# bdaiinstitute/judo

Measured on AMD Instinct MI355X. Metric: rollouts/sec + plan-step ms, leap_cube MPPI 65536xH64, higher is better.
Workload: dtype f32

## Files before the change

include/judo_amd.h:

```cpp
#ifndef JUDO_AMD_H
#define JUDO_AMD_H

#include <stddef.h>
#include <stdint.h>

#ifdef __cplusplus
extern "C" {
#endif

typedef struct jh_model jh_model;

enum jh_status {
  JH_OK = 0,
  JH_ERR_INVALID = -1,
  JH_ERR_HIP = -2,
  JH_ERR_UNSUPPORTED = -3,
  JH_ERR_BLOB = -4
};

enum jh_task_kind { JH_TASK_CARTPOLE = 0, JH_TASK_CYLINDER_PUSH = 1, JH_TASK_LEAP_CUBE = 2, JH_TASK_FR3_PICK = 3 };
enum jh_spline_kind { JH_SPLINE_ZERO = 0, JH_SPLINE_LINEAR = 1, JH_SPLINE_CUBIC = 3 };

#define JH_MAX_TASK_PARAMS 32
#define JH_MAX_KNOT_DIM 512
// ... 14 lines not shown
int jh_model_set_contact_capacity(jh_model* m, int contacts);

int jh_model_build(const jh_model* m, int* out );

int jh_model_fr3_build(const jh_model* m, int* out );

int jh_model_trace_layout(const jh_model* m, int* out );
int jh_trace_gather(const float* rec_in , int k, int stride_in, int n_offset, int n_local, const float* trace , int row_floats,
                    int colmajor, float* rec_out , void* stream);

int jh_model_limits(const jh_model* m, int* out );
int jh_model_max_fused_knots(const jh_model* m, int H);
int jh_model_one_launch_max_knots(const jh_model* m, int H);
int jh_model_set_plan_step_launches(jh_model* m, int launches);
int jh_model_set_rollout_schedule(jh_model* m, int mode);

int jh_upload_async(void* dst_device, const void* src_host, size_t nbytes, void* stream);
int jh_download_wait(void* dst_host, const void* src_device, size_t nbytes, void* stream);
int jh_download_begin(void* dst_host, const void* src_device, size_t nbytes, void* stream);
int jh_download_end(void);

int jh_rollout_cost(const jh_model* m, const float* x0, const float* nominal, const float* noise, int ldn, const float* sigma,
                    const float* W, const float* ctrl_lo_hi, const float* task_params, int phase, int N, int n_offset, int H, int K,
                    float* costs, float* knots_out, void* stream);
int jh_rollout_cost_traced(const jh_model* m, const float* x0, const float* nominal, const float* noise, int ldn, const float* sigma,
                    const float* W, const float* ctrl_lo_hi, const float* task_params, int phase, int N, int n_offset, int H, int K,
                    float* costs, float* knots_out, float* trace , void* stream);

int jh_rollout_materialize(const jh_model* m, const float* x0, int x0_batched, const float* controls, int N, int H, float* states,
                           float* sensors, void* stream);
// ... 99 lines not shown
```

judo_amd/_lib.py:

```python

from __future__ import annotations

import ctypes as C
import os

_HERE = os.path.dirname(os.path.abspath(__file__))
LIB_PATH = os.environ.get("JUDO_AMD_LIB") or os.path.join(_HERE, "libjudo_amd.so")

_lib: C.CDLL | None = None

f32p = C.c_void_p

_SIGNATURES = {
    "jh_last_error": (C.c_char_p, []),
    "jh_version": (C.c_int, []),
    "jh_model_create": (C.c_int, [C.c_void_p, C.c_size_t, C.c_int, C.POINTER(C.c_void_p)]),
    "jh_model_destroy": (None, [C.c_void_p]),
    "jh_model_dims": (C.c_int, [C.c_void_p, C.POINTER(C.c_int)]),
    "jh_model_stats": (C.c_int, [C.c_void_p, C.POINTER(C.c_int), C.c_int]),
    "jh_model_set_kernel": (C.c_int, [C.c_void_p, C.c_int]),
    "jh_model_limits": (C.c_int, [C.c_void_p, C.POINTER(C.c_int)]),
    "jh_register_xcheck": (C.c_int, [C.c_void_p]),
    "jh_model_max_fused_knots": (C.c_int, [C.c_void_p, C.c_int]),
    "jh_model_one_launch_max_knots": (C.c_int, [C.c_void_p, C.c_int]),
    "jh_model_set_plan_step_launches": (C.c_int, [C.c_void_p, C.c_int]),
    "jh_model_set_rollout_schedule": (C.c_int, [C.c_void_p, C.c_int]),
    "jh_model_set_self_collision": (C.c_int, [C.c_void_p, C.c_int]),
    "jh_model_set_contact_capacity": (C.c_int, [C.c_void_p, C.c_int]),
    "jh_model_build": (C.c_int, [C.c_void_p, C.POINTER(C.c_int)]),
    "jh_model_fr3_build": (C.c_int, [C.c_void_p, C.POINTER(C.c_int)]),
    "jh_model_trace_layout": (C.c_int, [C.c_void_p, C.POINTER(C.c_int)]),
    "jh_trace_gather": (C.c_int, [C.c_void_p, C.c_int, C.c_int, C.c_int, C.c_int, C.c_void_p, C.c_int, C.c_int, C.c_void_p, C.c_void_p]),
    "jh_upload_async": (C.c_int, [C.c_void_p, C.c_void_p, C.c_size_t, C.c_void_p]),
    "jh_download_wait": (C.c_int, [C.c_void_p, C.c_void_p, C.c_size_t, C.c_void_p]),
    "jh_download_begin": (C.c_int, [C.c_void_p, C.c_void_p, C.c_size_t, C.c_void_p]),
    "jh_download_end": (C.c_int, []),
    "jh_rollout_cost": (C.c_int, [C.c_void_p, f32p, f32p, f32p, C.c_int, f32p, f32p, f32p, f32p, C.c_int, C.c_int, C.c_int, C.c_int, C.c_int, f32p, f32p, C.c_void_p]),
    "jh_rollout_cost_traced": (C.c_int, [C.c_void_p, f32p, f32p, f32p, C.c_int, f32p, f32p, f32p, f32p, C.c_int, C.c_int, C.c_int, C.c_int, C.c_int, f32p, f32p, f32p, C.c_void_p]),
    "jh_rollout_materialize": (C.c_int, [C.c_void_p, f32p, C.c_int, f32p, C.c_int, C.c_int, f32p, f32p, C.c_void_p]),
    "jh_task_reward": (C.c_int, [C.c_void_p, f32p, f32p, f32p, f32p, C.c_int, C.c_int, C.c_int, f32p, C.c_void_p]),
    "jh_noise_normal": (C.c_int, [C.c_ulonglong, C.c_uint, C.c_int, C.c_int, C.c_int, f32p, C.c_int, C.c_void_p]),
# ... 98 lines not shown
```

judo_amd/csrc/jh_api.hip:

```cpp
#include <algorithm>
#include <cmath>
#include <cstdlib>
#include <cstring>

#include "jh_internal.h"
#include "jh_update_dev.h"

static thread_local char g_err[512] = "";

void jh_set_error(const char* fmt, ...) {
  va_list ap;
  va_start(ap, fmt);
  vsnprintf(g_err, sizeof(g_err), fmt, ap);
  va_end(ap);
}

extern "C" const char* jh_last_error(void) { return g_err; }
extern "C" int jh_version(void) { return 100; }

static int image_cylinders(const jh_blob_header& h, const float* F, const int* I) {
  constexpr int HEADER = 24, BODY_I = 6, BODY_F = 32, BLOCK_I = 4, DOF_F = 20, ACT_I = 2, ACT_F = 8, GEOM_I = 2, GEOM_F = 20, GF_RBOUND = 15;
  if (h.nint < (uint32_t)HEADER || h.nfloat < (uint32_t)HEADER) return 0;
  const long NM = I[0], NBLK = I[1], nv = I[2], nu = I[4], NG = I[5];
  if (NM < 0 || NBLK < 0 || nv < 0 || nu < 0 || NG < 0) return 0;
// ... 106 lines not shown
    std::vector<int> I((const int*)(q + 4 * (size_t)h.nfloat), (const int*)(q + 4 * (size_t)h.nfloat) + h.nint);
    cylinders = image_cylinders(h, F.data(), I.data());
    if (cylinders < 0) return JH_ERR_BLOB;
    if (h.kind == JH_TASK_LEAP_CUBE && image_pair_tables(h, I.data()) < 0) return JH_ERR_BLOB;
    if (cylinders > 0 && h.kind != JH_TASK_LEAP_CUBE) { jh_set_error("model_create: %d cylinder geoms, and only the leap kernel has a cylinder build", cylinders); return JH_ERR_BLOB; }
    if (h.kind == JH_TASK_FR3_PICK) {
      arm_pairs = image_arm_pairs(h, I.data());
      if (arm_pairs < 0) return JH_ERR_BLOB;
    }
  }
  JH_HIP(hipSetDevice(device));
  jh_model* m = new jh_model();
  m->device = device; m->kind = (int)h.kind; m->nq = h.nq; m->nv = h.nv; m->nu = h.nu; m->ns = h.ns; m->ntaskparam = h.ntaskparam;
  m->nf = h.nfloat; m->ni = h.nint; m->d_f = nullptr; m->d_i = nullptr; m->d_stats = nullptr; m->kernel_gen = (h.kind == JH_TASK_LEAP_CUBE || h.kind == JH_TASK_FR3_PICK) ? 3 : 2; m->self_collision = 1; m->contact_capacity = cylinders > 0 ? 64 : 48; m->cylinders = cylinders; m->arm_pairs = arm_pairs;
  { const char* e = getenv("JUDO_AMD_ROLLOUT_SCHEDULE"); m->rollout_schedule = (e && (e[0] == '1' || e[0] == '2')) ? e[0] - '0' : 0; }
  { const char* e = getenv("JUDO_AMD_PLAN_STEP_LAUNCHES"); m->plan_step_launches = (e && e[0] == '2') ? 2 : 0; }
  const char* p = (const char*)blob + sizeof(h);
  m->h_f.assign((const float*)p, (const float*)p + h.nfloat);
  m->h_i.assign((const int*)(p + 4 * (size_t)h.nfloat), (const int*)(p + 4 * (size_t)h.nfloat) + h.nint);
  {
    hipMemPool_t pool = nullptr; int dev = 0;
    if (hipGetDevice(&dev) == hipSuccess && hipDeviceGetDefaultMemPool(&pool, dev) == hipSuccess && pool) {
      unsigned long long keep = ~0ull;
      (void)hipMemPoolSetAttribute(pool, hipMemPoolAttrReleaseThreshold, &keep);
    }
  }
  hipError_t e = hipMalloc(&m->d_f, 4 * (m->nf ? m->nf : 1));
  if (e == hipSuccess) e = hipMalloc(&m->d_i, 4 * (m->ni ? m->ni : 1));
  if (e == hipSuccess) e = hipMalloc(&m->d_stats, JH_NSTATS * sizeof(int));
  if (e == hipSuccess) e = hipMemset(m->d_stats, 0, JH_NSTATS * sizeof(int));
// ... 161 lines not shown
  const int k = JH_MAX_KNOT_DIM / (m->nu > 0 ? m->nu : 1), lds_k = jh_simple_one_launch_max_knots(m, H);
  return k < lds_k ? k : lds_k;
}

extern "C" int jh_model_set_plan_step_launches(jh_model* m, int launches) {
  JH_REQUIRE(m != nullptr && launches >= 0 && launches <= 2, "model_set_plan_step_launches: launches must be 0 (automatic), 1 or 2");
  JH_REQUIRE(launches != 1 || m->kind == JH_TASK_CARTPOLE || m->kind == JH_TASK_CYLINDER_PUSH, "model_set_plan_step_launches: only the closed-form models have a one-launch plan step");
  m->plan_step_launches = launches;
  return JH_OK;
}

extern "C" int jh_model_set_rollout_schedule(jh_model* m, int mode) {
  JH_REQUIRE(m != nullptr && mode >= 0 && mode <= 2, "model_set_rollout_schedule: mode must be 0 (automatic), 1 (static grid) or 2 (persistent waves wherever the kernel has them)");
  m->rollout_schedule = mode;
  return JH_OK;
}

extern "C" int jh_upload_async(void* dst, const void* src, size_t nbytes, void* stream) {
  JH_REQUIRE(dst && src, "upload_async: null pointer");
  JH_HIP(hipMemcpyAsync(dst, src, nbytes, hipMemcpyHostToDevice, (hipStream_t)stream));
  return JH_OK;
}

extern "C" int jh_download_wait(void* dst, const void* src, size_t nbytes, void* stream) {
  JH_REQUIRE(dst && src, "download_wait: null pointer");
  JH_HIP(hipMemcpyAsync(dst, src, nbytes, hipMemcpyDeviceToHost, (hipStream_t)stream));
  JH_HIP(hipStreamSynchronize((hipStream_t)stream));
  return JH_OK;
}

// ... 231 lines not shown
static int model_set_member(const char* who, const jh_model* m0, const jh_model* m, int b) {
  JH_REQUIRE(m != nullptr, "%s: member %d is a null pointer", who, b);
  if (m->kind == JH_TASK_FR3_PICK) { jh_set_error("%s: member %d is an fr3_pick model, which has no batched plan step (its phase is chosen per problem on the host)", who, b); return JH_ERR_UNSUPPORTED; }
  if (m->kind == JH_TASK_LEAP_CUBE && m->kernel_gen != 3) { jh_set_error("%s: member %d runs kernel_gen %d: only kernel generation 3 of the leap family has a batched launch", who, b, m->kernel_gen); return JH_ERR_UNSUPPORTED; }
  if (m->kind != JH_TASK_CARTPOLE && m->kind != JH_TASK_CYLINDER_PUSH && m->kind != JH_TASK_LEAP_CUBE) { jh_set_error("%s: member %d: no batched kernel for this model (kind %d)", who, b, m->kind); return JH_ERR_UNSUPPORTED; }
  if (m != m0) {
#define JH_SET_SAME(field, fmt)                                                                                                                                    \
  JH_REQUIRE(m->field == m0->field, "%s: member %d differs from the set's member 0 in " #field " (" fmt " against " fmt ")", who, b, m->field, m0->field)
    JH_SET_SAME(device, "%d"); JH_SET_SAME(kind, "%d"); JH_SET_SAME(nq, "%d"); JH_SET_SAME(nv, "%d"); JH_SET_SAME(nu, "%d"); JH_SET_SAME(ns, "%d"); JH_SET_SAME(ntaskparam, "%d");
    JH_SET_SAME(nf, "%zu"); JH_SET_SAME(ni, "%zu");
    if (const long w = int_sections_differ(m->h_i, m0->h_i); w >= 0) {
      jh_set_error("%s: member %d differs from the set's member 0 in the int section h_i (word %ld: %d against %d): topology, pair lists and lane lists are one for the launch", who, b, w, m->h_i[w], m0->h_i[w]);
      return JH_ERR_INVALID;
    }
    JH_SET_SAME(kernel_gen, "%d"); JH_SET_SAME(contact_capacity, "%d"); JH_SET_SAME(cylinders, "%d"); JH_SET_SAME(self_collision, "%d"); JH_SET_SAME(rollout_schedule, "%d");
    JH_SET_SAME(plan_step_launches, "%d");
#undef JH_SET_SAME
  }
  JH_REQUIRE(m->h_f.size() == m->nf && m->d_f, "%s: member %d has no float section of nf = %zu floats", who, b, m->nf);
  if (m->kind == JH_TASK_LEAP_CUBE) {
    const bool ok = m->cylinders > 0 ? jh_engine5_accepts_cyl(m) : m->contact_capacity > 48 ? jh_engine5_accepts_cap64(m) : jh_engine5_accepts(m);
    if (!ok) {
      jh_set_error("%s: member %d: the leap kernel does not accept this image (dimensions, table sizes, or h_f: the cube's inertia must be isotropic)", who, b);
      return JH_ERR_UNSUPPORTED;
    }
  }
  return JH_OK;
}

static int model_set_upload(jh_model_set* s, int b, const jh_model* m) {
// ... 156 lines not shown
```

judo_amd/csrc/jh_engine_v5.hip:

```cpp
#include <cstddef>
#include <type_traits>

#include "jh_coop.h"

using namespace jh_eng;
using namespace jh_coop;

namespace {

#ifdef JH_V5_WAVESTAMP
__device__ unsigned long long* g_wavestamp = nullptr;
__device__ int g_wavestamp_cap = 0;
#endif

constexpr int G = 16, RPW = 4, WAVE = 64;
constexpr int NCH = 4, NLK = 4;

constexpr int LSMAX = 16;
constexpr int WAVES_PER_EU = 2;
constexpr int WAVES_PER_BLOCK = 4;
constexpr int BFS = 33;
constexpr int PAS = 9;
constexpr int RSPAD = 4;
constexpr int C3PAD = 278;
constexpr int NSLDS = 3;
constexpr double BIGPROB = 0.999999;
constexpr int CVX_STOP_NM = 1000;
#define OPAQUE(x) asm volatile("" : "+v"(x))
#define WSYNC() do { __builtin_amdgcn_fence(__ATOMIC_RELEASE, "wavefront"); __builtin_amdgcn_wave_barrier(); __builtin_amdgcn_fence(__ATOMIC_ACQUIRE, "wavefront"); } while (0)
#ifndef JH_V5_NSLOT
#define JH_V5_NSLOT 2
#endif
#ifndef JH_V5_NSBIG
#define JH_V5_NSBIG 3
#endif
#ifndef JH_V5_CYL
#define JH_V5_CYL 0
#endif
constexpr int GCYL = 5;
constexpr int NSLOT = JH_V5_NSLOT;
constexpr int NSBIG = JH_V5_NSBIG;
constexpr int NCP = 16 * (NSBIG < NSLDS ? NSBIG : NSLDS);
constexpr int NCAP = 16 * NSBIG;
// ... 280 lines not shown
    if (rem != 0 && elig == 0) ok = false;
    if (elig != 0) maxlev = st;
#pragma unroll
    for (int a = 0; a < NCH; a++) if (((elig >> a) & 1) && a == c) { level = st; parent = pr[a]; }
    rem &= ~elig;
  }
  return ok;
}

template <bool MATERIALIZE, int WPB, bool SELF, bool PERSIST = false, bool BATCH = false>
__global__ __launch_bounds__(WAVE * WPB, WAVES_PER_EU) void k_leap_v5(const float* __restrict__ gF, const int* __restrict__ gI, const float* __restrict__ x0, int x0_batched,
                                                   const float* __restrict__ nominal, const float* __restrict__ noise, int ldn,
                                                   const float* __restrict__ sigma, const float* __restrict__ W, const float* __restrict__ lohi,
                                                   const float* __restrict__ tp, int N, int n_offset, int H, int K, float* __restrict__ costs,
                                                   float* __restrict__ knots_out, const float* __restrict__ controls, float* __restrict__ states,
                                                   float* __restrict__ sensors, int* __restrict__ stats, int dshift_, float* __restrict__ trace, float* __restrict__ ovf_all, unsigned* __restrict__ head,
                                                   long long batch_blk, long long batch_noise, long long batch_image) {
  static_assert(!BATCH || (!MATERIALIZE && !PERSIST), "batched launches are fused launches on the static grid");
  if constexpr (BATCH) {
    const long long pb = blockIdx.y;
    x0 += pb * batch_blk; nominal += pb * batch_blk; sigma += pb * batch_blk; lohi += pb * batch_blk; tp += pb * batch_blk;
    noise += pb * batch_noise; costs += pb * N; gF += pb * batch_image;
    if (trace) trace += pb * N * H * 15;
    if (NOVF > 0 && ovf_all) ovf_all += pb * N * (NOVF * POOL_F);
  }
  __shared__ RS sRS[RPW * WPB];
  __shared__ float sBody[16 * BFS];
  __shared__ float sTp[16];
  __shared__ float sGeomF[MAXG * GEOM_F];
  __shared__ int sGeomI[MAXG * GEOM_I];
  __shared__ int sLaneG[16 * MAXLG];
  __shared__ float sLane[16 * LC_N];
  __shared__ int sBP[SELF ? 2 * MAXBP : 4];
  __shared__ int sBG[SELF ? 2 * NBC : 4];
  __shared__ float sBB[SELF ? NBC * 8 : 4];
  __shared__ int sGrp[WPB];
  const int dshift = PERSIST ? 0 : dshift_;
#ifdef JH_V5_WAVESTAMP
  const unsigned long long ws_entry = wall_clock64(); unsigned long long ws_staged = ws_entry;
#endif
  const int tid = threadIdx.x, wv = tid >> 6, lane = tid & 63, r = lane >> 4;
  int l = lane & 15, c = l >> 2, s = l & 3;
  RS& S = sRS[wv * RPW + r];
  const int nmI = gI[0], nblkI = gI[1], nuI = gI[4], ngI = gI[5], nsiteI = gI[6], nsI = gI[7], oRef = gI[18];
  const int oBodyF = HEADER_F, oDofF = oBodyF + nmI * BODY_F, oActF = oDofF + gI[2] * DOF_F, oGeomF = oActF + nuI * ACT_F, oSiteF = oGeomF + ngI * GEOM_F;
  const int oGeomI = HEADER_I + nmI * BODY_I + nblkI * BLOCK_I + nuI * ACT_I, oSiteI = oGeomI + ngI * GEOM_I;
  const int oLane = gI[11], lgm = gI[12];
  const int oBP = gI[15], oBS = gI[16], nBP = gI[17], oBG = oBP + 2 * nBP;
  for (int i = tid; i < 16 * BODY_F; i += WAVE * WPB) sBody[(i / BODY_F) * BFS + i % BODY_F] = gF[oBodyF + BODY_F + i];
  for (int i = tid; i < ngI * GEOM_F; i += WAVE * WPB) sGeomF[i] = gF[oGeomF + i];
  for (int i = tid; i < ngI * GEOM_I; i += WAVE * WPB) sGeomI[i] = gI[oGeomI + i];
// ... 10 lines not shown
    lc[LC_DAMP] = df[DF_DAMP]; lc[LC_KVD] = df[DF_KV]; lc[LC_FL] = df[DF_FL]; lc[LC_FB] = df[DF_FB]; lc[LC_FD] = df[DF_FD]; lc[LC_INVW] = df[DF_INVW];
    lc[LC_LIMITED] = df[DF_LIMITED]; lc[LC_LO] = df[DF_LO]; lc[LC_HI] = df[DF_HI]; lc[LC_LK] = df[DF_LK]; lc[LC_LB] = df[DF_LB];
    for (int k = 0; k < 5; k++) lc[LC_SI + k] = df[DF_SOLIMP + k];
    lc[LC_KP] = af[AF_KP]; lc[LC_KV] = af[AF_KV]; lc[LC_CLIM] = af[AF_CLIM]; lc[LC_CLO] = af[AF_CLO]; lc[LC_CHI] = af[AF_CHI];
    lc[LC_IMCK] = l < 6 ? 1.f / (l < 3 ? gF[HF_CMASS] : gF[HF_CINERTIA + (l < 3 ? 0 : l - 3)]) : 0.f;
  }
  const float* lc = sLane + l * LC_N;
  int grp = blockIdx.x * WPB + wv;
  const int ngroups = (N + RPW - 1) / RPW;
  if constexpr (PERSIST) {
    __syncthreads();
#ifdef JH_V5_WAVESTAMP
    ws_staged = wall_clock64();
#endif
  }
  for (; !PERSIST || grp < ngroups;) {
  if constexpr (PERSIST) { if (lane == 0) sGrp[wv] = grp; }
#ifdef JH_V5_WAVESTAMP
  const unsigned long long ws_start = wall_clock64();
#endif
  const int n = (grp << (2 - dshift)) + (r >> dshift);
  const bool live = n < N && (r & ((1 << dshift) - 1)) == 0;
  const int nc = n < N ? n : N - 1;
  const float h = gF[HF_DT], impratio = gF[HF_IMPRATIO], tol = gF[HF_TOL], lstol = gF[HF_LSTOL]; const int cap = (int)gF[HF_MAXITER];
  const float grav[3] = {gF[HF_GRAV], gF[HF_GRAV + 1], gF[HF_GRAV + 2]};
  const float cmass = gF[HF_CMASS], cI[3] = {gF[HF_CINERTIA], gF[HF_CINERTIA + 1], gF[HF_CINERTIA + 2]};
  const float chs[3] = {gF[HF_CSIZE], gF[HF_CSIZE + 1], gF[HF_CSIZE + 2]}, crb = gF[HF_CRBOUND], ctran = gF[HF_CTRAN];
  const float cK = gF[HF_CK], cB = gF[HF_CB];
  float csi[5]; for (int k = 0; k < 5; k++) csi[k] = gF[HF_SOLIMP + k];
  const float mck = (l < 3 ? cmass : (l == 3 ? cI[0] : (l == 4 ? cI[1] : (l == 5 ? cI[2] : 0.f))));
  float q, qd, qc[7], vc[6];
  {
    const float* xi = x0 + ((MATERIALIZE && x0_batched) ? (size_t)nc * NX : 0);
    for (int k = 0; k < 7; k++) qc[k] = xi[k];
    for (int k = 0; k < 6; k++) vc[k] = xi[NQ + k];
    q = xi[7 + l]; qd = xi[NQ + 6 + l];
  }
  auto knot_at = [&](int k, int ll, int ncc) -> float {
    const int i = k * NU + ll;
    float v = nominal[i];
    if (n_offset + ncc != 0) v = fmaf(sigma[i], noise[(size_t)i * ldn + ncc], v);
    return jh_clampf(v, lohi[ll], lohi[NU + ll]);
  };
  if (!MATERIALIZE) {
    if (knots_out && live) for (int k = 0; k < K; k++) knots_out[(size_t)(k * NU + l) * ldn + n] = knot_at(k, l, nc);
  }
  S.ws[6 + l] = 0.f; if (l < 6) S.ws[l] = 0.f;
  if (l < 4) S.cmd[l] = l == 0 ? cmass : (l == 1 ? cI[0] : (l == 2 ? cI[1] : cI[2]));
  int n_iters = 0, n_maxed = 0, n_wave_iters = 0;
  float acc = 0.f;
#ifdef JH_V5_TICKS
  long long cyc[16] = {0, 0, 0, 0, 0, 0, 0, 0, 0, 0, 0, 0, 0, 0, 0, 0}, t0 = clock64();
#define V5_TICK(slot) { long long t__ = clock64(); cyc[slot] += t__ - t0; t0 = t__; }
#else
#define V5_TICK(slot)
#endif
#ifdef JH_V5_COUNT
  int cnt_dense = 0, cnt_it = 0, cnt_l2 = 0, cnt_bp = 0, cnt_hh = 0, cnt_cls[4] = {0, 0, 0, 0};
  enum { CB_SPH = 34, CB_SPHMAX, CB_BOXMAX, CB_L1PAIRPASS, CB_L1LISTPASS, CB_TRIPS, CB_BPAIRS, CB_T, CB_COMBOPASS, CB_CUBEBOX, CB_CUBEBOXLANES, CB_MSPH, CB_MBOX, CB_MT, CB_NOSPH, CB_ONEA, CB_ONEB,
         CB_OWNTRIPS, CB_SPHOVER, CB_FEWSPH, CB_TSAFE, CB_TDROP };
#define V5_CADD(k, v) do { if (stats) atomicAdd(stats + (k), (int)(v)); } while (0)
#define V5_CMAX(k, v) do { if (stats) atomicMax(stats + (k), (int)(v)); } while (0)
#endif
  if constexpr (PERSIST) WSYNC();
  else {
    __syncthreads();
#ifdef JH_V5_WAVESTAMP
    ws_staged = wall_clock64();
#endif
  }

  for (int hh = 0; hh < H; hh++) {
    OPAQUE(l); c = l >> 2; s = l & 3;
    const float* lc = sLane + l * LC_N;
    float u;
    if (MATERIALIZE) u = controls[((size_t)nc * H + hh) * NU + l];
    else {
      u = 0.f;
      {
        int lo_ = lane; OPAQUE(lo_);
        const int g_ = PERSIST ? sGrp[wv] : (int)(blockIdx.x * WPB + wv);
        const int n_ = (g_ << (2 - dshift)) + ((lo_ >> 4) >> dshift), nc_ = n_ < N ? n_ : N - 1;
        for (int k = 0; k < K; k++) u = fmaf(W[hh * K + k], knot_at(k, l, nc_), u);
      }
    }
    float Mrow[NLK], fs_own, a0_own;
    {
// ... 1059 lines not shown
      }
      float nn = rsqrtf(qc[3] * qc[3] + qc[4] * qc[4] + qc[5] * qc[5] + qc[6] * qc[6]);
      qc[3] *= nn; qc[4] *= nn; qc[5] *= nn; qc[6] *= nn;
    }
    V5_TICK(7)
    if (MATERIALIZE) {
      if (states && live) {
        float* o = states + ((size_t)nc * H + hh) * NX;
        o[7 + l] = q; o[NQ + 6 + l] = qd;
        if (l < 7) o[l] = qc[l];
        if (l < 6) o[NQ + l] = vc[l];
      }
    } else acc += leap_step_cost(sTp, qc);
    WSYNC();
  }
#ifdef JH_V5_COUNT
  if (stats) { if (lane == 0) { atomicAdd(stats + 24, cnt_dense); atomicAdd(stats + 25, cnt_it); atomicAdd(stats + 26, cnt_l2); atomicAdd(stats + 28, H); } if (l == 0 && live) { atomicAdd(stats + 27, cnt_bp); atomicAdd(stats + 29, cnt_hh); for (int k = 0; k < 4; k++) atomicAdd(stats + 30 + k, cnt_cls[k]); } }
#endif
#ifdef JH_V5_TICKS
  if (lane == 0 && stats) { for (int k = 0; k < 8; k++) atomicAdd((unsigned long long*)(stats + 4) + k, (unsigned long long)cyc[k]);
                            for (int k = 0; k < 16; k++) atomicAdd((unsigned long long*)(stats + 384) + k, (unsigned long long)cyc[k]); }
#endif
  if (!MATERIALIZE && live && l == 0) costs[n] = acc / (float)H;
  if (stats && live && l == 0) { if (n_maxed) atomicAdd(stats + 1, n_maxed); atomicAdd(stats + 2, n_iters); atomicAdd(stats + 3, H); }
  if (stats && lane == 0 && live) { atomicAdd(stats + 20, n_wave_iters); atomicAdd(stats + 21, H); }
#ifdef JH_V5_WAVESTAMP
  if (lane == 0 && g_wavestamp && grp < g_wavestamp_cap) {
    unsigned long long* w = g_wavestamp + (size_t)grp * 6;
    w[0] = ((unsigned long long)blockIdx.x << 32) | ((unsigned long long)wv << 8) | (__smid() & 0xff); w[1] = ws_entry; w[2] = ws_staged; w[3] = ws_start; w[4] = wall_clock64(); w[5] = 1;
  }
#endif
  if constexpr (!PERSIST) break;
  else {
    int t = 0;
    if (lane == 0) t = (int)atomicAdd(head, 1u);
    grp = (int)(gridDim.x * WPB) + __builtin_amdgcn_readfirstlane(t);
  }
  }
}

bool model_is_leap(const jh_model* m) {
  return m->kind == JH_TASK_LEAP_CUBE && m->nq == 23 && m->nv == 22 && m->nu == 16 && (m->ns == NS || (m->ns == NS_CALTECH && m->h_i.size() > 18 && m->h_i[18] > 0)) && m->h_i.size() > 17 &&
         m->h_i[0] == 17 && m->h_i[1] == 4 && m->h_i[11] > 0 && m->h_i[5] <= MAXG && m->h_i[12] <= MAXLG && m->h_i[17] <= MAXBP
         && m->h_f.size() > (size_t)HF_CINERTIA + 2 && m->h_f[HF_CINERTIA] == m->h_f[HF_CINERTIA + 1] && m->h_f[HF_CINERTIA] == m->h_f[HF_CINERTIA + 2]
         ;
}

int device_cus(const jh_model* m) {
  int v = 0;
  return (hipDeviceGetAttribute(&v, hipDeviceAttributeMultiprocessorCount, m->device) == hipSuccess && v > 0) ? v : 256;
}
// ... 6 lines not shown
#ifdef JH_V5_WAVESTAMP
extern "C" int JH_V5_NAME(jh_v5_wavestamp_buffer)(unsigned long long* buf, int groups) {
  JH_HIP(hipMemcpyToSymbol(HIP_SYMBOL(g_wavestamp), &buf, sizeof(buf)));
  JH_HIP(hipMemcpyToSymbol(HIP_SYMBOL(g_wavestamp_cap), &groups, sizeof(groups)));
  return JH_OK;
}
#endif
int JH_V5_NAME(jh_engine5_rollout_cost)(const jh_model* m, const float* x0, const float* nominal, const float* noise, int ldn, const float* sigma, const float* W,
                            const float* lohi, const float* tp, int N, int n_offset, int H, int K, float* costs, float* knots_out, float* trace, hipStream_t st) {
  if (!model_is_leap(m)) { jh_set_error("rollout_cost: the cooperative engine kernel is instantiated for leap_cube only"); return JH_ERR_UNSUPPORTED; }
  if ((m->cylinders > 0) != (JH_V5_CYL != 0)) { jh_set_error("rollout_cost: an image with cylinder geoms runs on the cylinder build of the leap kernel and no other image does (%d cylinders)", m->cylinders); return JH_ERR_UNSUPPORTED; }
  const int dshift = jh_latency_shift(N, RPW); const int per_block = (RPW >> dshift) * WAVES_PER_BLOCK;
  int grid = (N + per_block - 1) / per_block;
  bool persist = dshift == 0 && m->rollout_schedule != 1; int slots = 0;
  if (persist) { slots = 2 * device_cus(m); persist = m->rollout_schedule == 2 || grid > slots; }
  const size_t ovf_bytes = NOVF > 0 ? (size_t)N * NOVF * POOL_F * sizeof(float) : 0;
  float* scratch = nullptr; float* ovf = nullptr; unsigned* head = nullptr;
  if (ovf_bytes > 0 || persist) scratch = jh_launch_scratch(m, ovf_bytes + (persist ? 16 : 0), st, ovf_bytes > 0);
  if (scratch && persist && hipMemsetAsync(scratch, 0, 16, st) != hipSuccess) { (void)hipGetLastError(); persist = false; }
  if (!scratch) persist = false;
  if (persist) { head = (unsigned*)scratch; if (grid > slots) grid = slots; }
  if (scratch && ovf_bytes > 0) ovf = scratch + (head ? 4 : 0);
#define JH_V5_LAUNCH_COST(SELF_, PERSIST_)                                                                                                                                        \
  hipLaunchKernelGGL((k_leap_v5<false, WAVES_PER_BLOCK, SELF_, PERSIST_>), dim3(grid), dim3(WAVE * WAVES_PER_BLOCK), 0, st, m->d_f, m->d_i, x0, 0, nominal, noise, ldn, sigma, W, \
                     lohi, tp, N, n_offset, H, K, costs, knots_out, (const float*)nullptr, (float*)nullptr, (float*)nullptr, m->d_stats, dshift, trace, ovf, head, 0ll, 0ll, 0ll)
  if (m->self_collision && m->h_i[17] > 0) { if (persist) JH_V5_LAUNCH_COST(true, true); else JH_V5_LAUNCH_COST(true, false); }
  else { if (persist) JH_V5_LAUNCH_COST(false, true); else JH_V5_LAUNCH_COST(false, false); }
#undef JH_V5_LAUNCH_COST
  return jh_launch_done(scratch, st);
}

int JH_V5_NAME(jh_engine5_materialize)(const jh_model* m, const float* x0, int x0_batched, const float* controls, int N, int H, float* states, float* sensors,
                           hipStream_t st) {
  if (!model_is_leap(m)) { jh_set_error("rollout_materialize: the cooperative engine kernel is instantiated for leap_cube only"); return JH_ERR_UNSUPPORTED; }
  if ((m->cylinders > 0) != (JH_V5_CYL != 0)) { jh_set_error("rollout_materialize: an image with cylinder geoms runs on the cylinder build of the leap kernel and no other image does (%d cylinders)", m->cylinders); return JH_ERR_UNSUPPORTED; }
  const int dshift = jh_latency_shift(N, RPW); const int per_block = (RPW >> dshift) * WAVES_PER_BLOCK;
  int grid = (N + per_block - 1) / per_block;
  float* ovf = nullptr;
  if (NOVF > 0) ovf = jh_launch_scratch(m, (size_t)N * NOVF * POOL_F * sizeof(float), st);
  if (m->self_collision && m->h_i[17] > 0)
    hipLaunchKernelGGL((k_leap_v5<true, WAVES_PER_BLOCK, true>), dim3(grid), dim3(WAVE * WAVES_PER_BLOCK), 0, st, m->d_f, m->d_i, x0, x0_batched, (const float*)nullptr, (const float*)nullptr, 0,
                       (const float*)nullptr, (const float*)nullptr, (const float*)nullptr, (const float*)nullptr, N, 0, H, 0, (float*)nullptr, (float*)nullptr,
                       controls, states, sensors, m->d_stats, dshift, (float*)nullptr, ovf, (unsigned*)nullptr, 0ll, 0ll, 0ll);
  else
    hipLaunchKernelGGL((k_leap_v5<true, WAVES_PER_BLOCK, false>), dim3(grid), dim3(WAVE * WAVES_PER_BLOCK), 0, st, m->d_f, m->d_i, x0, x0_batched, (const float*)nullptr, (const float*)nullptr, 0,
                       (const float*)nullptr, (const float*)nullptr, (const float*)nullptr, (const float*)nullptr, N, 0, H, 0, (float*)nullptr, (float*)nullptr,
                       controls, states, sensors, m->d_stats, dshift, (float*)nullptr, ovf, (unsigned*)nullptr, 0ll, 0ll, 0ll);
  return jh_launch_done(ovf, st);
}

int JH_V5_NAME(jh_engine5_rollout_cost_batch)(const jh_model* m, const float* images, long long image_stride, const int* ints, int B, const float* x0, const float* nominal, const float* sigma, const float* lohi, const float* tp, long long blk_stride,
                                  const float* noise, int ldn, long long noise_stride, const float* W, int N, int H, int K, float* costs, float* trace, hipStream_t st) {
  if (!model_is_leap(m)) { jh_set_error("plan_step_batch: the cooperative engine kernel is instantiated for leap_cube only"); return JH_ERR_UNSUPPORTED; }
  if ((m->cylinders > 0) != (JH_V5_CYL != 0)) { jh_set_error("plan_step_batch: an image with cylinder geoms runs on the cylinder build of the leap kernel and no other image does (%d cylinders)", m->cylinders); return JH_ERR_UNSUPPORTED; }
  JH_REQUIRE((long long)B * N <= 0x7fffffffll, "plan_step_batch: B * N = %lld rollouts exceed one launch", (long long)B * N);
  const int dshift = jh_latency_shift(B * N, RPW); const int per_block = (RPW >> dshift) * WAVES_PER_BLOCK;
  const int grid = (N + per_block - 1) / per_block;
  const size_t ovf_bytes = NOVF > 0 ? (size_t)B * N * NOVF * POOL_F * sizeof(float) : 0;
  float* ovf = ovf_bytes > 0 ? jh_launch_scratch(m, ovf_bytes, st) : nullptr;
#define JH_V5_LAUNCH_BATCH(SELF_)                                                                                                                                                  \
  hipLaunchKernelGGL((k_leap_v5<false, WAVES_PER_BLOCK, SELF_, false, true>), dim3(grid, B), dim3(WAVE * WAVES_PER_BLOCK), 0, st, images, ints, x0, 0, nominal, noise, ldn, sigma, W, \
                     lohi, tp, N, 0, H, K, costs, (float*)nullptr, (const float*)nullptr, (float*)nullptr, (float*)nullptr, m->d_stats, dshift, trace, ovf, (unsigned*)nullptr, blk_stride, noise_stride, image_stride)
  if (m->self_collision && m->h_i[17] > 0) JH_V5_LAUNCH_BATCH(true); else JH_V5_LAUNCH_BATCH(false);
#undef JH_V5_LAUNCH_BATCH
  return jh_launch_done(ovf, st);
}

bool JH_V5_NAME(jh_engine5_accepts)(const jh_model* m) { return model_is_leap(m) && (m->cylinders > 0) == (JH_V5_CYL != 0); }
```

judo_amd/csrc/jh_internal.h:

```cpp
#pragma once

#include <hip/hip_runtime.h>

#include <cstdarg>
#include <cstdint>
#include <cstdio>
#include <vector>

#include "judo_amd.h"
#include "judo_amd_xcheck.h"

#define JH_BLOB_MAGIC 0x314D484Au
#define JH_BLOB_VERSION 1u
#define JH_NSTATS 512
constexpr int JH_PT_SLOT = 19, JH_PT_MAX = 4, JH_PT_I = 9, JH_PT_LEN = 1 + JH_PT_MAX * JH_PT_I;

struct jh_blob_header {
  uint32_t magic, version, kind, nq, nv, nu, ns, ntaskparam, nfloat, nint;
  uint32_t reserved[6];
};

struct jh_model {
  int device, kind, nq, nv, nu, ns, ntaskparam;
  size_t nf, ni;
  float* d_f;
  int* d_i;
  int kernel_gen;
  int contact_capacity;
  int cylinders;
  int arm_pairs;
  int self_collision;
  int rollout_schedule;
  int plan_step_launches;
  mutable int one_launch_steps = 0;
  mutable int ovf_fallbacks = 0;
  int* d_stats;
  std::vector<float> h_f;
  std::vector<int> h_i;
};

void jh_set_error(const char* fmt, ...);

inline float* jh_launch_scratch(const jh_model* m, size_t bytes, hipStream_t st, bool overflow_rows = true) {
  hipMemPool_t pool = nullptr; void* p = nullptr;
  if (hipDeviceGetDefaultMemPool(&pool, m->device) == hipSuccess && pool && hipMallocFromPoolAsync(&p, bytes, pool, st) == hipSuccess) return (float*)p;
  (void)hipGetLastError();
  if (!overflow_rows) return nullptr;
// ... 124 lines not shown
```

judo_amd/device.py:

```python

from __future__ import annotations

import ctypes as C
import os

import numpy as np
import torch

from judo_amd import _lib
from judo_amd.models import layout, load_description, pack_model


def require_gpu() -> torch.device:
    if not torch.cuda.is_available():
        raise RuntimeError("judo_amd needs an MI355X (HIP device): torch.cuda.is_available() is False and there is no CPU fallback")
    return torch.device("cuda", torch.cuda.current_device())


_raw_stream = getattr(torch._C, "_cuda_getCurrentRawStream", None)


def current_stream_ptr() -> int:
    if _raw_stream is not None:
        return int(_raw_stream(torch.cuda.current_device()))
# ... 113 lines not shown
            self._max_knots_cache[H] = k
        return k

    def one_launch_max_knots_at(self, H: int) -> int:
        k = int(_lib.lib().jh_model_one_launch_max_knots(self.handle, int(H)))
        if k < 0:
            _lib.check(k, "jh_model_one_launch_max_knots")
        return k

    def set_plan_step_launches(self, launches: int) -> None:
        _lib.check(_lib.lib().jh_model_set_plan_step_launches(self.handle, int(launches)), "jh_model_set_plan_step_launches")

    def set_rollout_schedule(self, mode: int) -> None:
        _lib.check(_lib.lib().jh_model_set_rollout_schedule(self.handle, int(mode)), "jh_model_set_rollout_schedule")

    def stats(self, reset: bool = True) -> dict:
        out = (C.c_int * 8)()
        _lib.check(_lib.lib().jh_model_stats(self.handle, out, int(reset)), "jh_model_stats")
        u = [v & 0xFFFFFFFF for v in out]
        return {"contact_overflow": u[0], "newton_cap_hits": u[1], "newton_iters": u[2], "steps": u[3], "wave_newton_iters": u[4], "wave_steps": u[5], "overflow_pool_fallbacks": u[6], "one_launch_plan_steps": u[7]}

    def __del__(self) -> None:
        try:
            if getattr(self, "handle", None):
                _lib.lib().jh_model_destroy(self.handle)
                self.handle = None
        except Exception:
            pass


# ... 37 lines not shown
```

Baseline: 1.289 million.

## Slice persistent rollout work along the horizon with parked state hand-offs

Splits each rollout group's horizon into several slices that are queued as separate work units on the persistent-wave schedule. A later slice resumes from state parked in global memory by the earlier slice, and if that hand-off is not ready it recomputes the prefix. The aim is finer-grained load balancing across waves and less tail imbalance at large N. In exchange it adds global-memory park/restore traffic, flag synchronisation, possible redundant recomputation, and a larger scratch allocation.

After: 1.340 million, median of 6. +4.0%, better.

```diff
diff --git a/include/judo_amd.h b/include/judo_amd.h
--- a/include/judo_amd.h
+++ b/include/judo_amd.h
@@ -52,6 +52,9 @@
 int jh_model_one_launch_max_knots(const jh_model* m, int H);
 int jh_model_set_plan_step_launches(jh_model* m, int launches);
 int jh_model_set_rollout_schedule(jh_model* m, int mode);
+int jh_model_set_rollout_slices(jh_model* m, int slices, int max_workgroups, int flags);
+int jh_model_last_rollout_slices(const jh_model* m);
+int jh_model_recomputed_units(jh_model* m);
 
 int jh_upload_async(void* dst_device, const void* src_host, size_t nbytes, void* stream);
 int jh_download_wait(void* dst_host, const void* src_device, size_t nbytes, void* stream);
diff --git a/judo_amd/_lib.py b/judo_amd/_lib.py
--- a/judo_amd/_lib.py
+++ b/judo_amd/_lib.py
@@ -25,6 +25,9 @@
     "jh_model_one_launch_max_knots": (C.c_int, [C.c_void_p, C.c_int]),
     "jh_model_set_plan_step_launches": (C.c_int, [C.c_void_p, C.c_int]),
     "jh_model_set_rollout_schedule": (C.c_int, [C.c_void_p, C.c_int]),
+    "jh_model_set_rollout_slices": (C.c_int, [C.c_void_p, C.c_int, C.c_int, C.c_int]),
+    "jh_model_last_rollout_slices": (C.c_int, [C.c_void_p]),
+    "jh_model_recomputed_units": (C.c_int, [C.c_void_p]),
     "jh_model_set_self_collision": (C.c_int, [C.c_void_p, C.c_int]),
     "jh_model_set_contact_capacity": (C.c_int, [C.c_void_p, C.c_int]),
     "jh_model_build": (C.c_int, [C.c_void_p, C.POINTER(C.c_int)]),
diff --git a/judo_amd/csrc/jh_api.hip b/judo_amd/csrc/jh_api.hip
--- a/judo_amd/csrc/jh_api.hip
+++ b/judo_amd/csrc/jh_api.hip
@@ -144,6 +144,7 @@
   m->device = device; m->kind = (int)h.kind; m->nq = h.nq; m->nv = h.nv; m->nu = h.nu; m->ns = h.ns; m->ntaskparam = h.ntaskparam;
   m->nf = h.nfloat; m->ni = h.nint; m->d_f = nullptr; m->d_i = nullptr; m->d_stats = nullptr; m->kernel_gen = (h.kind == JH_TASK_LEAP_CUBE || h.kind == JH_TASK_FR3_PICK) ? 3 : 2; m->self_collision = 1; m->contact_capacity = cylinders > 0 ? 64 : 48; m->cylinders = cylinders; m->arm_pairs = arm_pairs;
   { const char* e = getenv("JUDO_AMD_ROLLOUT_SCHEDULE"); m->rollout_schedule = (e && (e[0] == '1' || e[0] == '2')) ? e[0] - '0' : 0; }
+  { const char* e = getenv("JUDO_AMD_ROLLOUT_SLICES"); const int v = e ? atoi(e) : 0; m->rollout_slices = (v >= 1 && v <= 64) ? v : 0; }
   { const char* e = getenv("JUDO_AMD_PLAN_STEP_LAUNCHES"); m->plan_step_launches = (e && e[0] == '2') ? 2 : 0; }
   const char* p = (const char*)blob + sizeof(h);
   m->h_f.assign((const float*)p, (const float*)p + h.nfloat);
@@ -335,6 +336,26 @@
   JH_REQUIRE(m != nullptr && mode >= 0 && mode <= 2, "model_set_rollout_schedule: mode must be 0 (automatic), 1 (static grid) or 2 (persistent waves wherever the kernel has them)");
   m->rollout_schedule = mode;
   return JH_OK;
+}
+
+extern "C" int jh_model_set_rollout_slices(jh_model* m, int slices, int max_workgroups, int flags) {
+  JH_REQUIRE(m != nullptr && slices >= 0 && slices <= 64, "model_set_rollout_slices: slices must be 0 (automatic) or 1 .. 64");
+  JH_REQUIRE(max_workgroups >= 0, "model_set_rollout_slices: max_workgroups must be 0 (the resident slots) or a positive cap on the queue's grid");
+  JH_REQUIRE((flags & ~1) == 0, "model_set_rollout_slices: flags has bit 0 (every hand-off counts as missed) and no other");
+  m->rollout_slices = slices; m->rollout_max_workgroups = max_workgroups; m->rollout_slice_flags = flags;
+  return JH_OK;
+}
+
+extern "C" int jh_model_last_rollout_slices(const jh_model* m) {
+  JH_REQUIRE(m != nullptr, "model_last_rollout_slices: null model");
+  return __atomic_load_n(&m->last_rollout_slices, __ATOMIC_RELAXED);
+}
+
+extern "C" int jh_model_recomputed_units(jh_model* m) {
+  JH_REQUIRE(m != nullptr, "model_recomputed_units: null model");
+  int v = 0;
+  JH_HIP(hipMemcpy(&v, m->d_stats + 56, sizeof(int), hipMemcpyDeviceToHost));
+  return v;
 }
 
 extern "C" int jh_upload_async(void* dst, const void* src, size_t nbytes, void* stream) {
@@ -596,6 +617,7 @@
       return JH_ERR_INVALID;
     }
     JH_SET_SAME(kernel_gen, "%d"); JH_SET_SAME(contact_capacity, "%d"); JH_SET_SAME(cylinders, "%d"); JH_SET_SAME(self_collision, "%d"); JH_SET_SAME(rollout_schedule, "%d");
+    JH_SET_SAME(rollout_slices, "%d"); JH_SET_SAME(rollout_max_workgroups, "%d"); JH_SET_SAME(rollout_slice_flags, "%d");
     JH_SET_SAME(plan_step_launches, "%d");
 #undef JH_SET_SAME
   }
diff --git a/judo_amd/csrc/jh_engine_v5.hip b/judo_amd/csrc/jh_engine_v5.hip
--- a/judo_amd/csrc/jh_engine_v5.hip
+++ b/judo_amd/csrc/jh_engine_v5.hip
@@ -27,6 +27,13 @@
 constexpr double BIGPROB = 0.999999;
 constexpr int CVX_STOP_NM = 1000;
 #define OPAQUE(x) asm volatile("" : "+v"(x))
+constexpr int PARK_F = 5 * 64;
+constexpr int STAT_RECOMPUTED = 56;
+#ifndef JH_V5_AUTO_SLICES
+#define JH_V5_AUTO_SLICES 4
+#endif
+#define PARK_LD(p) __hip_atomic_load((p), __ATOMIC_RELAXED, __HIP_MEMORY_SCOPE_AGENT)
+#define PARK_ST(p, v) __hip_atomic_store((p), (v), __ATOMIC_RELAXED, __HIP_MEMORY_SCOPE_AGENT)
 #define WSYNC() do { __builtin_amdgcn_fence(__ATOMIC_RELEASE, "wavefront"); __builtin_amdgcn_wave_barrier(); __builtin_amdgcn_fence(__ATOMIC_ACQUIRE, "wavefront"); } while (0)
 #ifndef JH_V5_NSLOT
 #define JH_V5_NSLOT 2
@@ -337,15 +344,15 @@
                                                    const float* __restrict__ sigma, const float* __restrict__ W, const float* __restrict__ lohi,
                                                    const float* __restrict__ tp, int N, int n_offset, int H, int K, float* __restrict__ costs,
                                                    float* __restrict__ knots_out, const float* __restrict__ controls, float* __restrict__ states,
-                                                   float* __restrict__ sensors, int* __restrict__ stats, int dshift_, float* __restrict__ trace, float* __restrict__ ovf_all, unsigned* __restrict__ head,
-                                                   long long batch_blk, long long batch_noise, long long batch_image) {
+                                                   float* __restrict__ sensors, int* __restrict__ stats_, int dshift_, float* __restrict__ trace, float* __restrict__ ovf_all_, unsigned* __restrict__ head,
+                                                   long long batch_blk, long long batch_noise, long long batch_image, unsigned* pflags, int slices_) {
   static_assert(!BATCH || (!MATERIALIZE && !PERSIST), "batched launches are fused launches on the static grid");
   if constexpr (BATCH) {
     const long long pb = blockIdx.y;
     x0 += pb * batch_blk; nominal += pb * batch_blk; sigma += pb * batch_blk; lohi += pb * batch_blk; tp += pb * batch_blk;
     noise += pb * batch_noise; costs += pb * N; gF += pb * batch_image;
     if (trace) trace += pb * N * H * 15;
-    if (NOVF > 0 && ovf_all) ovf_all += pb * N * (NOVF * POOL_F);
+    if (NOVF > 0 && ovf_all_) ovf_all_ += pb * N * (NOVF * POOL_F);
   }
   __shared__ RS sRS[RPW * WPB];
   __shared__ float sBody[16 * BFS];
@@ -358,6 +365,7 @@
   __shared__ int sBG[SELF ? 2 * NBC : 4];
   __shared__ float sBB[SELF ? NBC * 8 : 4];
   __shared__ int sGrp[WPB];
+  __shared__ int sUnit[4 * WPB];
   const int dshift = PERSIST ? 0 : dshift_;
 #ifdef JH_V5_WAVESTAMP
   const unsigned long long ws_entry = wall_clock64(); unsigned long long ws_staged = ws_entry;
@@ -398,14 +406,45 @@
     ws_staged = wall_clock64();
 #endif
   }
-  for (; !PERSIST || grp < ngroups;) {
-  if constexpr (PERSIST) { if (lane == 0) sGrp[wv] = grp; }
+  int unit = grp;
+  const int nsl = PERSIST ? max(1, min(slices_ & 0xff, H)) : 1, nunits = nsl * ngroups;
+  float* park = (float*)(pflags + ((nunits + 3) & ~3));
+  bool again = false;
+  float q, qd, qc[7], vc[6], acc;
 #ifdef JH_V5_WAVESTAMP
-  const unsigned long long ws_start = wall_clock64();
+  unsigned long long ws_start = 0;
+#endif
+  for (; !PERSIST || unit < nunits;) {
+  bool resumed = false, prefix = false; int hh0 = 0;
+  if constexpr (PERSIST) if (again) {
+    unit = __builtin_amdgcn_readfirstlane(sUnit[4 * wv + 3]); grp = unit % ngroups; hh0 = __builtin_amdgcn_readfirstlane(sUnit[4 * wv + 1]);
+    const int h1 = __builtin_amdgcn_readfirstlane(sUnit[4 * wv + 2]);
+    WSYNC();
+    if (lane == 0) sUnit[4 * wv] = h1;
+  }
+  if constexpr (PERSIST) if (!again) {
+    grp = unit % ngroups;
+    const int sl = unit / ngroups, h0 = sl * H / nsl, h1 = (sl + 1) * H / nsl;
+    if (sl > 0) {
+      unsigned f = 0;
+      if (lane == 0 && !(slices_ & 0x100)) f = __hip_atomic_load(pflags + (unit - ngroups), __ATOMIC_ACQUIRE, __HIP_MEMORY_SCOPE_AGENT);
+      resumed = __builtin_amdgcn_readfirstlane(f) != 0;
+      if (resumed) { __builtin_amdgcn_fence(__ATOMIC_ACQUIRE, "agent"); hh0 = h0; }
+      prefix = !resumed;
+    }
+    if (lane == 0) { sGrp[wv] = grp; sUnit[4 * wv] = (sl == 0 || resumed) ? h1 : h0; sUnit[4 * wv + 1] = h0; sUnit[4 * wv + 2] = h1; sUnit[4 * wv + 3] = unit; }
+  }
+#ifdef JH_V5_WAVESTAMP
+  if (!PERSIST || !again) ws_start = wall_clock64();
 #endif
   const int n = (grp << (2 - dshift)) + (r >> dshift);
   const bool live = n < N && (r & ((1 << dshift) - 1)) == 0;
   const int nc = n < N ? n : N - 1;
+  int* stats = stats_; float* ovf_all = ovf_all_;
+  if constexpr (PERSIST) if (prefix) {
+    stats = nullptr;
+    if (NOVF > 0 && ovf_all_) ovf_all = ovf_all_ + ((long long)N + (long long)(blockIdx.x * WPB + wv) * RPW + r - nc) * (NOVF * POOL_F);
+  }
   const float h = gF[HF_DT], impratio = gF[HF_IMPRATIO], tol = gF[HF_TOL], lstol = gF[HF_LSTOL]; const int cap = (int)gF[HF_MAXITER];
   const float grav[3] = {gF[HF_GRAV], gF[HF_GRAV + 1], gF[HF_GRAV + 2]};
   const float cmass = gF[HF_CMASS], cI[3] = {gF[HF_CINERTIA], gF[HF_CINERTIA + 1], gF[HF_CINERTIA + 2]};
@@ -413,8 +452,7 @@
   const float cK = gF[HF_CK], cB = gF[HF_CB];
   float csi[5]; for (int k = 0; k < 5; k++) csi[k] = gF[HF_SOLIMP + k];
   const float mck = (l < 3 ? cmass : (l == 3 ? cI[0] : (l == 4 ? cI[1] : (l == 5 ? cI[2] : 0.f))));
-  float q, qd, qc[7], vc[6];
-  {
+  if (!PERSIST || !again) {
     const float* xi = x0 + ((MATERIALIZE && x0_batched) ? (size_t)nc * NX : 0);
     for (int k = 0; k < 7; k++) qc[k] = xi[k];
     for (int k = 0; k < 6; k++) vc[k] = xi[NQ + k];
@@ -427,12 +465,20 @@
     return jh_clampf(v, lohi[ll], lohi[NU + ll]);
   };
   if (!MATERIALIZE) {
-    if (knots_out && live) for (int k = 0; k < K; k++) knots_out[(size_t)(k * NU + l) * ldn + n] = knot_at(k, l, nc);
-  }
-  S.ws[6 + l] = 0.f; if (l < 6) S.ws[l] = 0.f;
+    if (knots_out && live && (!PERSIST || unit < ngroups)) for (int k = 0; k < K; k++) knots_out[(size_t)(k * NU + l) * ldn + n] = knot_at(k, l, nc);
+  }
+  if (!PERSIST || !again) { S.ws[6 + l] = 0.f; if (l < 6) S.ws[l] = 0.f; }
   if (l < 4) S.cmd[l] = l == 0 ? cmass : (l == 1 ? cI[0] : (l == 2 ? cI[1] : cI[2]));
   int n_iters = 0, n_maxed = 0, n_wave_iters = 0;
-  float acc = 0.f;
+  if (!PERSIST || !again) acc = 0.f;
+  if constexpr (PERSIST) if (resumed) {
+    float* pk = park + (size_t)(unit - ngroups) * PARK_F; const int r16 = lane & 48;
+    q = PARK_LD(pk + lane); qd = PARK_LD(pk + 64 + lane); S.ws[6 + l] = PARK_LD(pk + 128 + lane);
+    for (int k = 0; k < 7; k++) qc[k] = PARK_LD(pk + 192 + r16 + k);
+    for (int k = 0; k < 6; k++) vc[k] = PARK_LD(pk + 199 + r16 + k);
+    acc = PARK_LD(pk + 205 + r16);
+    if (l < 6) S.ws[l] = PARK_LD(pk + 256 + lane);
+  }
 #ifdef JH_V5_TICKS
   long long cyc[16] = {0, 0, 0, 0, 0, 0, 0, 0, 0, 0, 0, 0, 0, 0, 0, 0}, t0 = clock64();
 #define V5_TICK(slot) { long long t__ = clock64(); cyc[slot] += t__ - t0; t0 = t__; }
@@ -454,7 +500,8 @@
 #endif
   }
 
-  for (int hh = 0; hh < H; hh++) {
+  const int hend = PERSIST ? __builtin_amdgcn_readfirstlane(sUnit[4 * wv]) : H;
+  for (int hh = hh0; hh < hend; hh++) {
     OPAQUE(l); c = l >> 2; s = l & 3;
     const float* lc = sLane + l * LC_N;
     float u;
@@ -1544,19 +1591,34 @@
     } else acc += leap_step_cost(sTp, qc);
     WSYNC();
   }
+  if constexpr (PERSIST) {
+    again = __builtin_amdgcn_readfirstlane(sUnit[4 * wv]) < __builtin_amdgcn_readfirstlane(sUnit[4 * wv + 2]);
+    if (again) { if (lane == 0 && stats_) atomicAdd(stats_ + STAT_RECOMPUTED, 1); continue; }
+  }
+  int usteps = H; bool last = true;
+  if constexpr (PERSIST) { const int h0 = __builtin_amdgcn_readfirstlane(sUnit[4 * wv + 1]), h1 = __builtin_amdgcn_readfirstlane(sUnit[4 * wv + 2]); usteps = h1 - h0; last = h1 >= H; unit = __builtin_amdgcn_readfirstlane(sUnit[4 * wv + 3]); }
 #ifdef JH_V5_COUNT
-  if (stats) { if (lane == 0) { atomicAdd(stats + 24, cnt_dense); atomicAdd(stats + 25, cnt_it); atomicAdd(stats + 26, cnt_l2); atomicAdd(stats + 28, H); } if (l == 0 && live) { atomicAdd(stats + 27, cnt_bp); atomicAdd(stats + 29, cnt_hh); for (int k = 0; k < 4; k++) atomicAdd(stats + 30 + k, cnt_cls[k]); } }
+  if (stats) { if (lane == 0) { atomicAdd(stats + 24, cnt_dense); atomicAdd(stats + 25, cnt_it); atomicAdd(stats + 26, cnt_l2); atomicAdd(stats + 28, usteps); } if (l == 0 && live) { atomicAdd(stats + 27, cnt_bp); atomicAdd(stats + 29, cnt_hh); for (int k = 0; k < 4; k++) atomicAdd(stats + 30 + k, cnt_cls[k]); } }
 #endif
 #ifdef JH_V5_TICKS
   if (lane == 0 && stats) { for (int k = 0; k < 8; k++) atomicAdd((unsigned long long*)(stats + 4) + k, (unsigned long long)cyc[k]);
                             for (int k = 0; k < 16; k++) atomicAdd((unsigned long long*)(stats + 384) + k, (unsigned long long)cyc[k]); }
 #endif
-  if (!MATERIALIZE && live && l == 0) costs[n] = acc / (float)H;
-  if (stats && live && l == 0) { if (n_maxed) atomicAdd(stats + 1, n_maxed); atomicAdd(stats + 2, n_iters); atomicAdd(stats + 3, H); }
-  if (stats && lane == 0 && live) { atomicAdd(stats + 20, n_wave_iters); atomicAdd(stats + 21, H); }
+  if (!MATERIALIZE && live && l == 0 && last) costs[n] = acc / (float)H;
+  if (stats && live && l == 0) { if (n_maxed) atomicAdd(stats + 1, n_maxed); atomicAdd(stats + 2, n_iters); atomicAdd(stats + 3, usteps); }
+  if (stats && lane == 0 && live) { atomicAdd(stats + 20, n_wave_iters); atomicAdd(stats + 21, usteps); }
+  if constexpr (PERSIST) if (!last) {
+    float* pk = park + (size_t)unit * PARK_F;
+    float pv = l == 13 ? acc : 0.f;
+    for (int k = 0; k < 7; k++) if (l == k) pv = qc[k];
+    for (int k = 0; k < 6; k++) if (l == 7 + k) pv = vc[k];
+    PARK_ST(pk + lane, q); PARK_ST(pk + 64 + lane, qd); PARK_ST(pk + 128 + lane, S.ws[6 + l]); PARK_ST(pk + 192 + lane, pv); PARK_ST(pk + 256 + lane, l < 6 ? S.ws[l] : 0.f);
+    __threadfence();
+    if (lane == 0) __hip_atomic_store(pflags + unit, 1u, __ATOMIC_RELEASE, __HIP_MEMORY_SCOPE_AGENT);
+  }
 #ifdef JH_V5_WAVESTAMP
-  if (lane == 0 && g_wavestamp && grp < g_wavestamp_cap) {
-    unsigned long long* w = g_wavestamp + (size_t)grp * 6;
+  if (lane == 0 && g_wavestamp && (PERSIST ? unit : grp) < g_wavestamp_cap) {
+    unsigned long long* w = g_wavestamp + (size_t)(PERSIST ? unit : grp) * 6;
     w[0] = ((unsigned long long)blockIdx.x << 32) | ((unsigned long long)wv << 8) | (__smid() & 0xff); w[1] = ws_entry; w[2] = ws_staged; w[3] = ws_start; w[4] = wall_clock64(); w[5] = 1;
   }
 #endif
@@ -1564,7 +1626,7 @@
   else {
     int t = 0;
     if (lane == 0) t = (int)atomicAdd(head, 1u);
-    grp = (int)(gridDim.x * WPB) + __builtin_amdgcn_readfirstlane(t);
+    unit = (int)(gridDim.x * WPB) + __builtin_amdgcn_readfirstlane(t);
   }
   }
 }
@@ -1601,16 +1663,35 @@
   int grid = (N + per_block - 1) / per_block;
   bool persist = dshift == 0 && m->rollout_schedule != 1; int slots = 0;
   if (persist) { slots = 2 * device_cus(m); persist = m->rollout_schedule == 2 || grid > slots; }
-  const size_t ovf_bytes = NOVF > 0 ? (size_t)N * NOVF * POOL_F * sizeof(float) : 0;
+  const int ngroups = (N + RPW - 1) / RPW;
+  int slices = 1;
+  if (persist) {
+    slices = m->rollout_slices > 0 ? m->rollout_slices : (ngroups >= 2 * slots * WAVES_PER_BLOCK ? JH_V5_AUTO_SLICES : 1);
+    if (slices > H) slices = H;
+    if (slices < 1 || (long long)slices * ngroups > 0x7fffffffll) slices = 1;
+  }
+  int qgrid = grid;
+  if (persist) { if (qgrid > slots) qgrid = slots; if (m->rollout_max_workgroups > 0 && qgrid > m->rollout_max_workgroups) qgrid = m->rollout_max_workgroups; }
+  size_t flag_words = 0, queue_bytes = 0, ovf_bytes = 0;
   float* scratch = nullptr; float* ovf = nullptr; unsigned* head = nullptr;
-  if (ovf_bytes > 0 || persist) scratch = jh_launch_scratch(m, ovf_bytes + (persist ? 16 : 0), st, ovf_bytes > 0);
-  if (scratch && persist && hipMemsetAsync(scratch, 0, 16, st) != hipSuccess) { (void)hipGetLastError(); persist = false; }
+  for (;;) {
+    flag_words = slices > 1 ? (((size_t)slices * ngroups + 3) & ~(size_t)3) : 0;
+    const size_t park_floats = slices > 1 ? (size_t)(slices - 1) * ngroups * PARK_F : 0, own_rows = slices > 1 ? (size_t)qgrid * WAVES_PER_BLOCK * RPW : 0;
+    queue_bytes = persist ? 16 + (flag_words + park_floats) * sizeof(float) : 0;
+    ovf_bytes = NOVF > 0 ? ((size_t)N + own_rows) * NOVF * POOL_F * sizeof(float) : 0;
+    if (ovf_bytes > 0 || persist) scratch = jh_launch_scratch(m, ovf_bytes + queue_bytes, st, ovf_bytes > 0 && slices == 1);
+    if (scratch || slices == 1) break;
+    slices = 1;
+  }
+  if (scratch && persist && hipMemsetAsync(scratch, 0, 16 + flag_words * sizeof(unsigned), st) != hipSuccess) { (void)hipGetLastError(); persist = false; }
   if (!scratch) persist = false;
-  if (persist) { head = (unsigned*)scratch; if (grid > slots) grid = slots; }
-  if (scratch && ovf_bytes > 0) ovf = scratch + (head ? 4 : 0);
+  if (persist) { head = (unsigned*)scratch; grid = qgrid; } else slices = 1;
+  if (scratch && ovf_bytes > 0) ovf = scratch + (head ? queue_bytes / sizeof(float) : 0);
+  __atomic_store_n(&m->last_rollout_slices, persist ? slices : 0, __ATOMIC_RELAXED);
+  const int slices_arg = slices | ((m->rollout_slice_flags & 1) << 8);
 #define JH_V5_LAUNCH_COST(SELF_, PERSIST_)                                                                                                                                        \
   hipLaunchKernelGGL((k_leap_v5<false, WAVES_PER_BLOCK, SELF_, PERSIST_>), dim3(grid), dim3(WAVE * WAVES_PER_BLOCK), 0, st, m->d_f, m->d_i, x0, 0, nominal, noise, ldn, sigma, W, \
-                     lohi, tp, N, n_offset, H, K, costs, knots_out, (const float*)nullptr, (float*)nullptr, (float*)nullptr, m->d_stats, dshift, trace, ovf, head, 0ll, 0ll, 0ll)
+                     lohi, tp, N, n_offset, H, K, costs, knots_out, (const float*)nullptr, (float*)nullptr, (float*)nullptr, m->d_stats, dshift, trace, ovf, head, 0ll, 0ll, 0ll, head ? head + 4 : (unsigned*)nullptr, slices_arg)
   if (m->self_collision && m->h_i[17] > 0) { if (persist) JH_V5_LAUNCH_COST(true, true); else JH_V5_LAUNCH_COST(true, false); }
   else { if (persist) JH_V5_LAUNCH_COST(false, true); else JH_V5_LAUNCH_COST(false, false); }
 #undef JH_V5_LAUNCH_COST
@@ -1628,11 +1709,11 @@
   if (m->self_collision && m->h_i[17] > 0)
     hipLaunchKernelGGL((k_leap_v5<true, WAVES_PER_BLOCK, true>), dim3(grid), dim3(WAVE * WAVES_PER_BLOCK), 0, st, m->d_f, m->d_i, x0, x0_batched, (const float*)nullptr, (const float*)nullptr, 0,
                        (const float*)nullptr, (const float*)nullptr, (const float*)nullptr, (const float*)nullptr, N, 0, H, 0, (float*)nullptr, (float*)nullptr,
-                       controls, states, sensors, m->d_stats, dshift, (float*)nullptr, ovf, (unsigned*)nullptr, 0ll, 0ll, 0ll);
+                       controls, states, sensors, m->d_stats, dshift, (float*)nullptr, ovf, (unsigned*)nullptr, 0ll, 0ll, 0ll, (unsigned*)nullptr, 0);
   else
     hipLaunchKernelGGL((k_leap_v5<true, WAVES_PER_BLOCK, false>), dim3(grid), dim3(WAVE * WAVES_PER_BLOCK), 0, st, m->d_f, m->d_i, x0, x0_batched, (const float*)nullptr, (const float*)nullptr, 0,
                        (const float*)nullptr, (const float*)nullptr, (const float*)nullptr, (const float*)nullptr, N, 0, H, 0, (float*)nullptr, (float*)nullptr,
-                       controls, states, sensors, m->d_stats, dshift, (float*)nullptr, ovf, (unsigned*)nullptr, 0ll, 0ll, 0ll);
+                       controls, states, sensors, m->d_stats, dshift, (float*)nullptr, ovf, (unsigned*)nullptr, 0ll, 0ll, 0ll, (unsigned*)nullptr, 0);
   return jh_launch_done(ovf, st);
 }
 
@@ -1647,7 +1728,7 @@
   float* ovf = ovf_bytes > 0 ? jh_launch_scratch(m, ovf_bytes, st) : nullptr;
 #define JH_V5_LAUNCH_BATCH(SELF_)                                                                                                                                                  \
   hipLaunchKernelGGL((k_leap_v5<false, WAVES_PER_BLOCK, SELF_, false, true>), dim3(grid, B), dim3(WAVE * WAVES_PER_BLOCK), 0, st, images, ints, x0, 0, nominal, noise, ldn, sigma, W, \
-                     lohi, tp, N, 0, H, K, costs, (float*)nullptr, (const float*)nullptr, (float*)nullptr, (float*)nullptr, m->d_stats, dshift, trace, ovf, (unsigned*)nullptr, blk_stride, noise_stride, image_stride)
+                     lohi, tp, N, 0, H, K, costs, (float*)nullptr, (const float*)nullptr, (float*)nullptr, (float*)nullptr, m->d_stats, dshift, trace, ovf, (unsigned*)nullptr, blk_stride, noise_stride, image_stride, (unsigned*)nullptr, 0)
   if (m->self_collision && m->h_i[17] > 0) JH_V5_LAUNCH_BATCH(true); else JH_V5_LAUNCH_BATCH(false);
 #undef JH_V5_LAUNCH_BATCH
   return jh_launch_done(ovf, st);
diff --git a/judo_amd/csrc/jh_internal.h b/judo_amd/csrc/jh_internal.h
--- a/judo_amd/csrc/jh_internal.h
+++ b/judo_amd/csrc/jh_internal.h
@@ -31,6 +31,8 @@
   int arm_pairs;
   int self_collision;
   int rollout_schedule;
+  int rollout_slices = 0, rollout_max_workgroups = 0, rollout_slice_flags = 0;
+  mutable int last_rollout_slices = 0;
   int plan_step_launches;
   mutable int one_launch_steps = 0;
   mutable int ovf_fallbacks = 0;
diff --git a/judo_amd/device.py b/judo_amd/device.py
--- a/judo_amd/device.py
+++ b/judo_amd/device.py
@@ -151,6 +151,18 @@
     def set_rollout_schedule(self, mode: int) -> None:
         _lib.check(_lib.lib().jh_model_set_rollout_schedule(self.handle, int(mode)), "jh_model_set_rollout_schedule")
 
+    def set_rollout_slices(self, slices: int = 0, max_workgroups: int = 0, flags: int = 0) -> None:
+        _lib.check(_lib.lib().jh_model_set_rollout_slices(self.handle, int(slices), int(max_workgroups), int(flags)), "jh_model_set_rollout_slices")
+
+    def last_rollout_slices(self) -> int:
+        return int(_lib.lib().jh_model_last_rollout_slices(self.handle))
+
+    def recomputed_units(self) -> int:
+        v = int(_lib.lib().jh_model_recomputed_units(self.handle))
+        if v < 0:
+            _lib.check(v, "jh_model_recomputed_units")
+        return v
+
     def stats(self, reset: bool = True) -> dict:
         out = (C.c_int * 8)()
         _lib.check(_lib.lib().jh_model_stats(self.handle, out, int(reset)), "jh_model_stats")
```
